# DavidSlayback/gym-po-taxi

Measured on AMD Instinct MI355X. Metric: env steps/sec (whole node), FourRooms 11x11 Hansen-4 at 1M envs, 1/2/4/8 GPUs, higher is better.
Workload: dtype int32; 1 GPU; configs[1]: FourRooms 11x11 (FR_MAP) Hansen-4 obs, 1048576 envs per GPU, MultistoryFourRoomsEnv(grid_z=1, obs_type='hansen'); envs_per_gpu=1048576, global_envs=1048576, rng_mode=numpy, parallelism=independent env shards x1, steps_per_launch_call=128, kernel_autotune=windowed

## Files before the change

### gym-po-taxi_amd/csrc/api.hip

```cpp
#include <stdarg.h>
#include <stdio.h>
#include <string.h>

#include <string>
#include <vector>

#include "gp_internal.h"

struct gp_env {
  int kind = 0;
  std::unique_ptr<EnvBackend> be;
};

static thread_local char g_err[1024] = "";

void gp_set_error(const char* fmt, ...) {
  va_list ap;
  va_start(ap, fmt);
  vsnprintf(g_err, sizeof(g_err), fmt, ap);
  va_end(ap);
}

const char* gp_derr_text(uint32_t flags) {
  static thread_local char buf[512];
// ... 184 lines not shown
  else if (!strcmp(key, "fault_block")) g_dbg.fault_block = (int)value;
  else if (!strcmp(key, "fused_tile")) g_dbg.fused_tile = (int)value;
  else if (!strcmp(key, "generic_kernels")) g_dbg.generic_kernels = value != 0;
  else if (!strcmp(key, "no_spw")) g_dbg.no_spw = value != 0;
  else if (!strcmp(key, "no_wgrid")) g_dbg.no_wgrid = value != 0;
  else if (!strcmp(key, "wg_halo")) g_dbg.wg_halo = (int)value;
  else if (!strcmp(key, "wg_bias")) g_dbg.wg_bias = (int)value;
  else if (!strcmp(key, "wg_tmode")) g_dbg.wg_tmode = (int)value;
  else if (!strcmp(key, "wg_kmax")) g_dbg.wg_kmax = (int)value;
  else if (!strcmp(key, "taxi_npg_min")) g_dbg.taxi_npg_min = (int)value;
  else if (!strcmp(key, "xg_min_envs")) g_dbg.xg_min_envs = (int)value;
  else if (!strcmp(key, "fused_step")) g_dbg.fused_step = value;
  else if (!strcmp(key, "wg_block_envs")) g_dbg.wg_block_envs = (int)value;
  else if (!strcmp(key, "wg_fill_simd")) g_dbg.wg_fill_simd = (int)value;
  else if (!strcmp(key, "wg_fill_wave")) g_dbg.wg_fill_wave = value;
  else if (!strcmp(key, "xg_ppt_min")) g_dbg.xg_ppt_min = (int)value;
  else if (!strcmp(key, "xg_spb_min")) g_dbg.xg_spb_min = (int)value;
  else if (!strcmp(key, "persist_bpc")) g_dbg.persist_bpc = (int)value;
  else if (!strcmp(key, "ctrl_lds_max")) g_dbg.ctrl_lds_max = (int)value;
  else if (!strcmp(key, "xg_graph")) gp_xg_graph_knob = (int)value;
  else {
    gp_set_error("gp_debug_set: unknown key '%s'", key);
    return GP_E_INVALID;
  }
  return GP_OK;
}
void gp_debug_reset(void) {
  g_dbg = GpDebugKnobs{};
  gp_xg_graph_knob = -1;
}
// ... 339 lines not shown
```

### gym-po-taxi_amd/csrc/gp_internal.h

```cpp
#pragma once
#include <cstring>
#include <memory>
#include <string>
#include <vector>

#include "../../include/gym_po_amd.h"
#include "gp_common.h"

struct RngHost {
  u128 state = 0, inc = 1;
  uint32_t has_u32 = 0, uinteger = 0;
};

std::vector<uint64_t> seed_sequence_u64(const std::vector<uint32_t>& entropy, const std::vector<uint32_t>& spawn_key,
                                        int n_words64);
RngHost pcg64_from_seed(const std::vector<uint32_t>& entropy, const std::vector<uint32_t>& spawn_key);
std::vector<double> argmax_multinomial_distribution(int m, int n);
std::vector<PcgJump> build_jump_tables(u128 inc);

struct GpDebugKnobs {
  int disable_fused = 0, no_staging = 0, xmode = 1, fault_block = -1;
  int fused_tile = 0;
  uint32_t spin_limit = 0;
  int generic_kernels = 0;
  int no_spw = 0;
  int no_wgrid = 0;
  int wg_halo = 0;
  int wg_bias = 0;
  int wg_tmode = 0;
  int wg_kmax = -1;
  int xg_min_envs = -1;
  int xg_ppt_min = -1;
  int xg_spb_min = -1;
  int taxi_npg_min = -1;
  int64_t fused_step = -1;
  int wg_block_envs = 0;
  int wg_fill_simd = 0;
  int64_t wg_fill_wave = 0;
  int ctrl_lds_max = -1;
  int persist_bpc = 0;
};
const GpDebugKnobs& gp_debug_knobs();

inline int persistent_grid(int ntiles, int cus, int occ) {
  const int forced = gp_debug_knobs().persist_bpc;
  const int bpc = forced > 0 ? forced : (occ < 1 ? 1 : (occ > 8 ? 8 : occ));
  const int g = cus * bpc;
  return ntiles < g ? (ntiles > 0 ? ntiles : 1) : g;
}

struct KernelTimer {
  bool on = false;
  std::vector<std::pair<hipEvent_t, hipEvent_t>> ev;
// ... 130 lines not shown
```

### gym-po-taxi_amd/csrc/grid.hip

```cpp
#include <stdarg.h>
#include <stdio.h>
#include <stdlib.h>
#include <string.h>

#include <algorithm>
#include <cmath>

#include "gp_ctrl.h"
#include "gp_internal.h"
#include "grid_shared.h"

namespace {

constexpr int TPB = 256;
constexpr int EPT = 4;
constexpr int EPB = TPB * EPT;
constexpr uint32_t SPIN_LIMIT = 1u << 24;
constexpr int MAX_TPB2 = 1024;
#ifndef WG_KMAX
#define WG_KMAX 24
#endif
#ifndef WG_FILL_WAVE
#define WG_FILL_WAVE 0xFFFF1111u
#endif
// ... 2513 lines not shown
  uint64_t philox_step = 0;
  std::vector<int32_t> cells;
  std::vector<uint16_t> goal_valid_h, agent_valid_h;
  DevBuf b_move, b_thr, b_gv, b_av, b_hbase, b_doff, b_hvec, b_t1, b_t2, b_coords, b_window, b_jt, b_lt4, b_lt2,
      b_tja, b_tjw, b_ae, b_goal, b_ctl, b_tcount, b_tlist, b_rflag, b_mslot, b_ftj, b_flt4, b_fjB, b_fslot, b_dbg, b_self, b_jt8,
      b_limg, b_ofix, b_avo;
  int fused_G = 0, fused_qpt = 0;
  int wg_G = 0, wg_E = 0, wg_NS = 0, wg_H = 0;
  int wg_kmax = WG_KMAX;
  int wg_kmax_default = WG_KMAX;
  size_t wg_lds = 0;
  int at_launches = 0, at_steps = 0;
  float at_ms[2] = {0.f, 0.f};
  WgParams wg{};
  std::vector<char> wg_img;
  DevBuf b_wgp, b_wlimg, b_wjlane, b_wjrej, b_wjblk, b_wslots, b_wjfirst;
  bool fused_stg = false;
  const uint64_t* rp_u = nullptr;
  const int32_t* rp_goal = nullptr;
  const int32_t* rp_agent = nullptr;

  int build(const gp_grid_config* cfg);
  int upload_rng();
  int refresh_lds_image();
  int seed(const RngHost& r, const uint32_t key[2]) override {
    rng = r;
    philox_key[0] = key[0];
    philox_key[1] = key[1];
    d.key0 = key[0];
    d.key1 = key[1];
    philox_step = 0;
// ... 6 lines not shown
  int get_rng_state(RngHost* r) override;
  int check() override;
  int device_error(uint32_t flags);
  int query(const char* key, int64_t* v) const override {
    if (!strcmp(key, "fused_blocks")) *v = fused_G;
    else if (!strcmp(key, "fused_tiles_per_block")) *v = fused_qpt;
    else if (!strcmp(key, "fused_staged")) *v = fused_stg ? 1 : 0;
    else if (!strcmp(key, "fused_spw")) *v = d.spw_on;
    else if (!strcmp(key, "fused_tile_envs")) *v = d.ftile;
    else if (!strcmp(key, "wgrid")) *v = wg_G > 0 ? 1 : 0;
    else if (!strcmp(key, "wgrid_blocks")) *v = wg_G;
    else if (!strcmp(key, "wgrid_block_envs")) *v = wg_E;
    else if (!strcmp(key, "wgrid_halo")) *v = wg_H;
    else if (!strcmp(key, "wgrid_kmax")) *v = wg_kmax;
    else if (!strcmp(key, "wgrid_lds")) *v = (int64_t)wg_lds;
    else if (!strcmp(key, "autotune_launches")) *v = at_launches;
    else if (!strcmp(key, "autotune_steps")) *v = at_steps;
    else if (!strcmp(key, "autotune_wgrid_ns")) *v = (int64_t)(at_ms[0] * 1e6f);
    else if (!strcmp(key, "autotune_fused_ns")) *v = (int64_t)(at_ms[1] * 1e6f);
    else if (!strcmp(key, "philox_step")) *v = (int64_t)philox_step;
    else if (!strcmp(key, "controller_nodes")) *v = ctrl.M;
    else if (!strcmp(key, "controller_lds")) *v = ctrl.M && ctrl.lds_off >= 0;
    else return EnvBackend::query(key, v);
    return GP_OK;
  }
  int reset(void* obs, hipStream_t s) override;
  int step(const void* act, void* obs, float* rew, uint8_t* term, uint8_t* trunc, hipStream_t s) override;
  int rollout(int K, const void* act, void* obs, float* rew, uint8_t* term, uint8_t* trunc, hipStream_t s) override;
  int get_state(void* a, void* b, void* c, void* dd, hipStream_t s) override {
    hipLaunchKernelGGL(grid_get_state, dim3((unsigned)((B + TPB - 1) / TPB)), dim3(TPB), 0, s, d, (int32_t*)a,
// ... 203 lines not shown
      E = e;
      break;
    }
  if (!E) return GP_OK;
  for (int c : ocell)
    if (c < INT32_MIN / 2 || c > INT32_MAX / 2) return GP_OK;
  const int H = dbg.wg_halo == 512 ? 512 : 256;
  const int nc = d.ncells, na = d.nact;
  WgLds L{};
  int off = 0;
  auto put = [&](int32_t& o, size_t bytes) {
    o = off;
    off += (int)((bytes + 15) / 16 * 16);
  };
  put(L.j32, sizeof(PcgJump) * 32);
  put(L.jt8, sizeof(PcgJump) * 512);
  put(L.move, (size_t)nc * na * 2);
  put(L.thr, (size_t)na * na * 8);
  put(L.ocell, (size_t)nc * 4);
  put(L.avalid, agent_valid_h.size() * 2);
  L.total = off;
  const size_t lds = (size_t)wg_dyn_bytes(L.total, E, H);
  if (!wgrid_fits(E / 512, na, lds)) return GP_OK;
  wg_img.assign((size_t)L.total, 0);
  memcpy(wg_img.data() + L.move, move.data(), move.size() * 2);
  std::vector<uint64_t> th(thr.size());
  for (size_t i = 0; i < thr.size(); ++i) th[i] = thr_on_u64(thr[i]);
  memcpy(wg_img.data() + L.thr, th.data(), th.size() * 8);
  memcpy(wg_img.data() + L.ocell, ocell.data(), ocell.size() * 4);
  memcpy(wg_img.data() + L.avalid, agent_valid_h.data(), agent_valid_h.size() * 2);
  wg_G = (int)(B / E);
  wg_E = E;
  wg_NS = E / 512;
  wg_H = H;
  wg_lds = lds;
  WgParams& w = wg;
  w.B = (int32_t)B;
// ... 32 lines not shown
      dv[v] = n >= 8 ? n - 16 : n;
      vsum += dv[v];
      vok = vok && base + dl[v & 3] + dv[v] >= 1;
    }
    if (vsum != 0 || !vok)
      for (int v = 0; v < 8; ++v) dv[v] = 0;
    int r = 0;
    for (int v = 0; v < 8; ++v) {
      w.fill_row0[v] = r;
      w.fill_rows[v] = base + dl[v & 3] + dv[v];
      r += w.fill_rows[v];
    }
  }
  w.wg_bias = dbg.wg_bias;
  w.tmode = dbg.wg_tmode;
  w.lds = L;
  int e;
  if ((e = b_wgp.alloc(sizeof(WgParams))) || (e = b_wlimg.alloc((size_t)L.total)) ||
      (e = b_wjlane.alloc(sizeof(PcgJump) * 1024)) || (e = b_wjrej.alloc(sizeof(PcgJump) * 64 * (size_t)wg_G)) ||
      (e = b_wjblk.alloc(sizeof(PcgJump) * 2 * (size_t)wg_G)) || (e = b_wslots.alloc(sizeof(uint64_t) * 4 * (size_t)wg_G)) ||
      (e = b_wjfirst.alloc(sizeof(PcgJump) * 1024)))
    return e;
  w.jfirst = b_wjfirst.as<PcgJump>();
  w.limg = b_wlimg.as<char>();
  w.jlane = b_wjlane.as<PcgJump>();
  w.jrej = b_wjrej.as<PcgJump>();
  w.jblk = b_wjblk.as<PcgJump>();
  w.slots = b_wslots.as<uint64_t>();
  return GP_OK;
}

int GridBackend::upload_wgrid() {
  const u128 inc = rng.inc;
  WgParams& w = wg;
  auto compose = [](const PcgJump& j2, const PcgJump& j1) {
    const u128 a = mk128(j2.a_hi, j2.a_lo) * mk128(j1.a_hi, j1.a_lo);
    const u128 c = mk128(j2.a_hi, j2.a_lo) * mk128(j1.c_hi, j1.c_lo) + mk128(j2.c_hi, j2.c_lo);
    return PcgJump{hi64(a), lo64(a), hi64(c), lo64(c)};
  };
  PcgJump* j32 = reinterpret_cast<PcgJump*>(wg_img.data() + w.lds.j32);
  PcgJump* jt8 = reinterpret_cast<PcgJump*>(wg_img.data() + w.lds.jt8);
  for (int i = 0; i < 32; ++i) j32[i] = pcg_jump_params((u128)i, inc);
  for (int i = 0; i < 256; ++i) {
    jt8[i] = pcg_jump_params((u128)i, inc);
    jt8[256 + i] = pcg_jump_params((u128)(256 * i), inc);
  }
  std::vector<PcgJump> jl(1024), jr((size_t)64 * wg_G), jb(2 * (size_t)wg_G);
  const PcgJump one = pcg_jump_params((u128)1, inc), j32s = pcg_jump_params((u128)32, inc);
  const PcgJump jBp1 = pcg_jump_params((u128)B + 1, inc);
  jl[1] = jBp1;
  for (int l = 1; l < 512; ++l) jl[2 * l + 1] = compose(j32s, jl[2 * (l - 1) + 1]);
  for (int v = 0; v < 8; ++v) {
    PcgJump x = pcg_jump_params((u128)(64 * w.fill_row0[v]), inc);
    for (int l = 0; l < 64; ++l) {
      jl[2 * (64 * v + l)] = x;
      x = compose(one, x);
    }
  }
  const PcgJump j62 = pcg_jump_params((u128)62, inc);
  PcgJump row = jBp1;
  for (int b = 0; b < wg_G; ++b) {
    PcgJump x = row;
    for (int l = 0; l < 64; ++l) {
      jr[(size_t)b * 64 + l] = x;
      x = compose(one, x);
    }
    row = compose(j62, row);
    jb[2 * b] = pcg_jump_params((u128)B + (u128)(b ? wg_E * b - wg_H : 0), inc);
    jb[2 * b + 1] = b ? pcg_jump_params((u128)(wg_E * b - wg_H + 1), inc) : PcgJump{0, 1, 0, 0};
  }
  w.jB = pcg_jump_params((u128)B, inc);
  w.jrow = pcg_jump_params((u128)64, inc);
  w.j512 = pcg_jump_params((u128)512, inc);
  std::vector<PcgJump> jf(1024);
  jf[0] = one;
  jf[512] = pcg_jump_params((u128)wg_H, inc);
  for (int l = 1; l < 512; ++l) {
    jf[l] = compose(one, jf[l - 1]);
    jf[512 + l] = compose(one, jf[512 + l - 1]);
  }
  w.jt64 = d.jt;
  w.dbg = d.dbg;
  w.ctl = d.ctl;
  w.mslot = d.mslot;
  w.ae = d.ae;
  GP_HIP_CHECK(hipMemcpy(b_wlimg.p, wg_img.data(), wg_img.size(), hipMemcpyHostToDevice));
  GP_HIP_CHECK(hipMemcpy(b_wjlane.p, jl.data(), jl.size() * sizeof(PcgJump), hipMemcpyHostToDevice));
  GP_HIP_CHECK(hipMemcpy(b_wjrej.p, jr.data(), jr.size() * sizeof(PcgJump), hipMemcpyHostToDevice));
  GP_HIP_CHECK(hipMemcpy(b_wjblk.p, jb.data(), jb.size() * sizeof(PcgJump), hipMemcpyHostToDevice));
  GP_HIP_CHECK(hipMemcpy(b_wjfirst.p, jf.data(), jf.size() * sizeof(PcgJump), hipMemcpyHostToDevice));
  GP_HIP_CHECK(hipMemcpy(b_wgp.p, &w, sizeof(WgParams), hipMemcpyHostToDevice));
  return GP_OK;
}

int GridBackend::get_rng_state(RngHost* r) {
  GP_HIP_CHECK(hipDeviceSynchronize());
  GridCtl c;
  GP_HIP_CHECK(hipMemcpy(&c, d.ctl, sizeof(c), hipMemcpyDeviceToHost));
  r->state = mk128(c.s_hi, c.s_lo);
  r->inc = mk128(c.inc_hi, c.inc_lo);
  r->has_u32 = c.has_u32;
  r->uinteger = c.uinteger;
  if (c.err) return device_error(c.err);
  return GP_OK;
// ... 737 lines not shown
```

### gym-po-taxi_amd/csrc/grid_shared.h

```cpp
#pragma once
#include "gp_common.h"

struct alignas(64) GridCtl {
  uint64_t s_hi, s_lo, inc_hi, inc_lo;
  uint32_t has_u32, uinteger;
  uint32_t epoch;
  uint32_t err;
  uint32_t b_total;
  uint32_t step;
  uint32_t fb_last;
  uint32_t wstep;
};

struct alignas(32) MetricSlot {
  double return_sum;
  unsigned long long episodes, length_sum, env_steps;
};

constexpr int WG_HMAX = 512;

struct WgLds {
  int32_t j32, jt8, move, thr, ocell, avalid, total;
};

struct WgParams {
  int32_t B, G, E, NS;
  int32_t nact, ncells, n_agent, goal;
  uint32_t thr_agent;
  int32_t time_limit, halo;
  float r_step, r_wall, r_goal;
  uint32_t spin_limit;
  int32_t fault_block;
  int32_t rw_words;
  int32_t fill_row0[8], fill_rows[8];
  int32_t wg_bias;
  int32_t tmode;
  WgLds lds;
  const char* limg;
  const PcgJump* jlane;
  const PcgJump* jrej;
  const PcgJump* jblk;
  const PcgJump* jfirst;
  const PcgJump* jt64;
  PcgJump jB, jrow, j512;
  GridCtl* ctl;
  MetricSlot* mslot;
  uint32_t* ae;
  uint64_t* slots;
  unsigned long long* dbg;
};

struct WgArgs {
  const WgParams* P;
  int32_t K;
  const int32_t* act;
  int32_t* obs;
  float* rew;
  uint8_t* term;
  uint8_t* trunc;
};

__host__ __device__ constexpr int wg_dyn_bytes(int tables, int E, int H) {
#ifndef WG_NSTG
#define WG_NSTG 3
#endif
  return tables + (E + 2 * H) * 8 + 2 * 512 * 16 + WG_NSTG * E * 4;
}
int wgrid_launch(const WgArgs& a, int NS, int NA, int G, size_t dyn_lds, hipStream_t s);
int wgrid_fits(int NS, int NA, size_t dyn_lds);
```

### gym-po-taxi_amd/csrc/wgrid.hip

```cpp
#include <stdint.h>

#include "gp_internal.h"
#include "grid_shared.h"

namespace {

#ifdef GP_STAMPS
constexpr int ST_STEPS = 24, ST_SLOTS = 42;
__shared__ unsigned long long g_stamp[32 * 32 + 8];
#define WSTAMP(P, k, i)                                                                                  \
  do {                                                                                                   \
    if ((threadIdx.x & 63) == 0 && (k) < ST_STEPS) {                                                     \
      unsigned long long t_;                                                                             \
      asm volatile("s_memrealtime %0\n\ts_waitcnt lgkmcnt(0)" : "=s"(t_)::"memory");                     \
      g_stamp[(k) * ST_SLOTS + (i)] = t_;                                                                \
    }                                                                                                    \
  } while (0)
#define LSTAMP(P, i)                                                                                     \
  do {                                                                                                   \
    if ((threadIdx.x & 63) == 0) {                                                                       \
      unsigned long long t_;                                                                             \
      asm volatile("s_memrealtime %0\n\ts_waitcnt lgkmcnt(0)" : "=s"(t_)::"memory");                     \
      g_stamp[32 * 32 + (i)] = t_;                                                                       \
    }                                                                                                    \
// ... 37 lines not shown
constexpr int NCAND = 512;
constexpr uint32_t CAND_W = 192;

struct WgShared {
  uint64_t mask[8][EW];
  uint32_t trans_done;
  uint32_t cs_done;
  uint32_t r2s_done;
  uint32_t fill_done;
  uint32_t res_done;
  uint32_t st_done;
  uint32_t sx_ready;
  uint32_t sy_ready;
  uint32_t cells_done;
  uint32_t pro;
  uint64_t sx[2][2];
  uint64_t sy[2][2];
  uint64_t rw[2][2];
  int32_t rw_off[2];
  uint32_t fix[2];
  uint32_t R, h, u, nrp;
  uint32_t cbase;
  uint32_t rp[MAXRP];
  uint16_t r2s[4096];
  uint16_t cand[NCAND];
};

__device__ __forceinline__ void lds_barrier() {
  __builtin_amdgcn_fence(__ATOMIC_RELEASE, "workgroup", "local");
  __builtin_amdgcn_s_barrier();
// ... 47 lines not shown
}

__host__ __device__ __forceinline__ uint64_t thr_on_u64(uint64_t t) {
  return t >= (1ull << 53) ? ~0ull : ((t << 11) | 0x7FFull);
}

template <int NA>
__device__ __forceinline__ int32_t action_row(int32_t a, uint32_t* derr) {
  if (action_out_of_range(a, NA)) flag_bad_action(derr);
  if (a < 0) a += NA;
  return min(max(a, 0), NA - 1) * NA * 8;
}

struct Tabs {
  const PcgJump* j32p;
  const PcgJump* jt8p;
  const int32_t* ocp;
  const uint16_t* avp;
  const PcgJump* jt64;
  int32_t halo;
  __device__ __forceinline__ Tabs(const char* d, const WgParams& P)
      : j32p(reinterpret_cast<const PcgJump*>(d + P.lds.j32)), jt8p(reinterpret_cast<const PcgJump*>(d + P.lds.jt8)),
        ocp(reinterpret_cast<const int32_t*>(d + P.lds.ocell)), avp(reinterpret_cast<const uint16_t*>(d + P.lds.avalid)),
        jt64(P.jt64), halo(P.halo) {}
  __device__ __forceinline__ const PcgJump& j32(uint32_t i) const { return j32p[i]; }
  __device__ __forceinline__ const PcgJump& jt8(uint32_t i) const { return jt8p[i]; }
  __device__ __forceinline__ int32_t ocell(uint32_t c) const { return ocp[c]; }
  __device__ __forceinline__ uint32_t avalid(uint32_t v) const { return avp[v]; }
};

__device__ __forceinline__ u128 load_cs(const uint64_t* CS, uint32_t j) {
  const ulonglong2 v = reinterpret_cast<const ulonglong2*>(CS)[j];
  return mk128(v.y, v.x);
}
__device__ __forceinline__ u128 draw_state(const Tabs& tb, const uint64_t* CS, uint32_t d) {
  return apply_jump(tb.j32(d & 31u), load_cs(CS, d >> 5));
}

__device__ __forceinline__ u128 jump_any(const Tabs& tb, u128 s, uint32_t n) {
  if (n < 65536u) {
    if (n & 255u) s = apply_jump(tb.jt8(n & 255u), s);
    if (n >> 8) s = apply_jump(tb.jt8(256u + (n >> 8)), s);
    return s;
  }
  return pcg_jump(tb.jt64, s, n);
}

__device__ __forceinline__ u128 rw_base(const Tabs& tb, const PcgJump& jb, u128 Sx, uint32_t used, int beta,
                                        int32_t& heff) {
  const int32_t H = tb.halo;
  if (beta == 0) {
    heff = min(H, (int32_t)used + 1);
    return apply_jump(jb, jump_any(tb, Sx, used + 1u - (uint32_t)heff));
  }
  heff = H;
  return apply_jump(jb, jump_any(tb, Sx, used + 1u));
}
// ... 57 lines not shown
#define WG_NSTG 3
#endif
#ifndef WG_EAGER_TAIL
#define WG_EAGER_TAIL 4
#endif
#ifndef WG_SUNROLL
#define WG_SUNROLL 2
#endif
constexpr int NSTG = WG_NSTG;
struct Lds {
  uint64_t* RW;
  uint64_t* CS0;
  char* stg0;
  __device__ __forceinline__ Lds(char* dyn, const WgParams& P, int E)
      : RW(reinterpret_cast<uint64_t*>(dyn + P.lds.total)),
        CS0(reinterpret_cast<uint64_t*>(dyn + P.lds.total + (size_t)(E + 2 * P.halo) * 8)),
        stg0(dyn + P.lds.total + (size_t)(E + 2 * P.halo) * 8 + 2 * 512 * 16) {}
  __device__ __forceinline__ char* stg(int k, int E) const { return stg0 + (size_t)(k % NSTG) * E * 4; }
  __device__ __forceinline__ uint64_t* CS(int k) const { return CS0 + (size_t)(k & 1) * 1024; }
};

__device__ __forceinline__ void list_slice(const WgParams& P, WgShared& sh, const Tabs& tb, const uint64_t* CS,
                                           uint32_t sigma, u128 Sy, uint32_t h, uint32_t u) {
  const int lane = threadIdx.x & 63;
  bool rlo = false, rhi = false;
  if (lane < SLICE) {
    const uint32_t d = 62u * sigma + (uint32_t)lane;
    const u128 s = d < 16384u ? draw_state(tb, CS, d) : pcg_jump(tb.jt64, Sy, d + 1u);
    const uint64_t x = pcg_output(s);
    rlo = lemire_rejected((uint32_t)x, (uint32_t)P.n_agent, P.thr_agent);
    rhi = lemire_rejected((uint32_t)(x >> 32), (uint32_t)P.n_agent, P.thr_agent);
  }
// ... 57 lines not shown
    uint64_t g[4];
    exchange(P, slots + (size_t)(r & 1u) * G, (ts << 6) | r, cnt, 0u, g);
    rtot += list_flagged(P, sh, tb, CS, g, r, Sy, h, u);
    covered += 124u * (uint32_t)G;
  }
  uint32_t wtot = 0;
  if (b) {
    uint32_t p = b - 1u;
    const uint32_t n = sh.nrp;
    for (uint32_t q = 0; q < n; ++q) p += sh.rp[q] <= p ? 1u : 0u;
    wtot = p + 1u;
  }
  return wtot;
}

template <int NS, int NA>
__device__ __forceinline__ void wg_ctrl(const WgParams& P, WgShared& sh, const Tabs& tb, const Lds& L, int K) {
  const int lane = threadIdx.x & 63, beta = (int)blockIdx.x, G = (int)gridDim.x;
  constexpr int E = NS * 512;
  GridCtl* C = P.ctl;
  u128 Sx = mk128(C->s_hi, C->s_lo);
  uint32_t h = C->has_u32, u = C->uinteger;
  uint32_t bprev = C->fb_last;
  uint32_t Rprev = (uint32_t)(((uint64_t)bprev * (uint64_t)blockIdx.x) / (uint64_t)gridDim.x);
  const uint32_t ts0 = C->wstep + 1u;
  const PcgJump jr = P.jrej[(size_t)beta * 64 + lane];
  const PcgJump jb = P.jblk[2 * beta], jpro = P.jblk[2 * beta + 1];
  const PcgJump jB = P.jB;
  const uint32_t nag = (uint32_t)P.n_agent, thra = P.thr_agent;
  const int32_t H = P.halo;
  const uint32_t bias = (uint32_t)P.wg_bias;
  const bool envcells = NS <= 2 && !(P.tmode & TM_CELLSWAP);
  uint32_t* derr = &C->err;
  lds_barrier();
  if (lane == 0 && (P.tmode & TM_OLDPRO)) {
    const u128 s = apply_jump(jpro, Sx);
    sh.rw[0][0] = hi64(s);
    sh.rw[0][1] = lo64(s);
    sh.rw_off[0] = beta == 0 ? 1 : H;
    lds_release();
    __hip_atomic_store(&sh.pro, 1u, __ATOMIC_RELAXED, __HIP_MEMORY_SCOPE_WORKGROUP);
  }
  LSTAMP(P, 1);
  for (int k = 0; k < K; ++k) {
    const uint32_t ts = ts0 + (uint32_t)k;
    if (lane == 0) {
      sh.sx[k & 1][0] = hi64(Sx);
      sh.sx[k & 1][1] = lo64(Sx);
      lds_release();
      __hip_atomic_store(&sh.sx_ready, (uint32_t)k + 1u, __ATOMIC_RELAXED, __HIP_MEMORY_SCOPE_WORKGROUP);
    }
    uint32_t rj = 0;
    if (lane < SLICE) {
      const uint64_t x = pcg_output(apply_jump(jr, Sx));
      rj = (lemire_rejected((uint32_t)x, nag, thra) ? 1u : 0u) + (lemire_rejected((uint32_t)(x >> 32), nag, thra) ? 1u : 0u);
    } else if (lane == SLICE && beta == 0 && h) {
      rj = lemire_rejected(u, nag, thra) ? 1u : 0u;
    }
    const uint32_t rejc = wave_sum(rj);
    WSTAMP(P, k, 6);
    lds_wait(&sh.trans_done, (uint32_t)EW * (uint32_t)(k + 1), derr);
    WSTAMP(P, k, 7);
    const uint32_t cb = wave_sum(lane < NS * EW ? (uint32_t)__builtin_popcountll(sh.mask[lane >> 3][lane & 7]) : 0u);
    uint64_t* slots = P.slots + (size_t)(ts & 1u) * 2 * G;
    publish(P, slots, ts << 6, rejc, cb);
    WSTAMP(P, k, 8);
    const u128 Sy = apply_jump(jB, Sx);
    uint32_t used_p, hp;
    words_to_draws(bprev + bias, h, used_p, hp);
    int32_t heff_p;
    const u128 Srw = rw_base(tb, jb, Sx, used_p, beta, heff_p);
    if (lane == 0) {
      sh.sy[k & 1][0] = hi64(Sy);
      sh.sy[k & 1][1] = lo64(Sy);
      sh.rw[(k + 1) & 1][0] = hi64(Srw);
      sh.rw[(k + 1) & 1][1] = lo64(Srw);
      lds_release();
      __hip_atomic_store(&sh.sy_ready, (uint32_t)k + 1u, __ATOMIC_RELAXED, __HIP_MEMORY_SCOPE_WORKGROUP);
    }
    const uint64_t* CS = L.CS(k);
    lds_wait(&sh.cs_done, (uint32_t)EW * (uint32_t)(k + 1), derr);
    const uint32_t d0 = min(Rprev > CAND_W + h ? (Rprev - CAND_W - h) >> 1 : 0u, 16384u - NCAND / 2);
    const uint32_t cbase = 2u * d0 + h;
    if (!(P.tmode & TM_NOCAND)) {
#pragma unroll
      for (int m = 0; m < NCAND / 128; ++m) {
        const uint32_t j = (uint32_t)(lane + 64 * m);
        const uint64_t x = pcg_output(draw_state(tb, CS, d0 + j));
        sh.cand[2 * j] = (uint16_t)tb.avalid(lemire_value((uint32_t)x, nag));
        sh.cand[2 * j + 1] = (uint16_t)tb.avalid(lemire_value((uint32_t)(x >> 32), nag));
      }
// ... 47 lines not shown
            cell = tb.avalid(lemire_value(word, nag));
          }
          st[2 * slot] = (uint16_t)cell;
        }
      }
    } else {
      const uint32_t wtot = ctrl_slow(P, sh, tb, CS, Sy, h, u, b, ts, g);
      words_to_draws(wtot, h, used, h2);
      if (lane == 0) {
        sh.R = R;
        sh.h = h;
        sh.u = u;
      }
    }
    int32_t off = heff_p + (int32_t)used - (int32_t)used_p;
    uint32_t fix = slow ? 1u : 0u;
    if (k + 1 < K && (off < 0 || off > 2 * H)) {
      int32_t heff;
      const u128 s = rw_base(tb, jb, Sx, used, beta, heff);
      off = heff;
      fix |= 2u;
      if (lane == 0) {
        sh.rw[(k + 1) & 1][0] = hi64(s);
        sh.rw[(k + 1) & 1][1] = lo64(s);
      }
    }
    if (lane == 0) {
      sh.rw_off[(k + 1) & 1] = off;
      sh.fix[k & 1] = fix;
      lds_release();
      __hip_atomic_store(&sh.cells_done, (uint32_t)k + 1u, __ATOMIC_RELAXED, __HIP_MEMORY_SCOPE_WORKGROUP);
    }
    WSTAMP(P, k, 10);
    Sx = jump_any(tb, Sy, used);
    if (used) u = (uint32_t)(pcg_output(Sx) >> 32);
    h = h2;
    bprev = b;
    Rprev = R;
    WSTAMP(P, k, 12);
  }
  LSTAMP(P, 3);
  if (beta == 0 && lane == 0) {
    C->s_hi = hi64(Sx);
    C->s_lo = lo64(Sx);
    C->has_u32 = h;
    C->uinteger = u;
    C->fb_last = bprev;
    C->wstep = ts0 + (uint32_t)K - 1u;
  }
}

struct Acc {
  uint32_t eps = 0, ngoal = 0, nwall = 0, lens = 0;
};

template <int NS>
__device__ __forceinline__ void wg_env_slow(const WgParams& P, WgShared& sh, const Tabs& tb, const uint64_t* CS,
                                            int k, char* stg, uint32_t dn, const uint32_t (&pre)[NS],
                                            const uint64_t (&bm)[NS], uint32_t (&ae)[NS]) {
  const int lg = threadIdx.x;
  const u128 Sy = mk128(sh.sy[k & 1][0], sh.sy[k & 1][1]);
  const uint32_t R = sh.R, h = sh.h, u = sh.u, n = sh.nrp;
#pragma unroll
// ... 45 lines not shown
    reinterpret_cast<uint16_t*>(stg)[2 * (s * 512 + lg)] = (uint16_t)cell;
    ae[s] = cell;
  }
}

__device__ __forceinline__ void fill_window(uint64_t* RW, const PcgJump& jl, const PcgJump& jrow, int fr0, int nrow,
                                            u128 base, int lane) {
  u128 s = apply_jump(jl, base);
  uint64_t* d = RW + fr0 * 64 + lane;
  for (int m = 0; m < nrow; ++m) {
    d[m * 64] = pcg_output(s);
    s = apply_jump(jrow, s);
  }
}

template <int NS, int NA>
__device__ __forceinline__ void wg_env(const WgParams& P, WgShared& sh, const Tabs& tb, const Lds& L, const char* dyn,
                                       const int32_t* __restrict__ act, int K, Acc& acc, int32_t* __restrict__ obs,
                                       float* __restrict__ rew, uint8_t* __restrict__ term,
                                       uint8_t* __restrict__ trunc) {
  const int lg = threadIdx.x, lane = lg & 63, w = lg >> 6;
  const int beta = (int)blockIdx.x, G = (int)gridDim.x;
  constexpr int E = NS * 512;
  const size_t B = (size_t)E * (size_t)G;
  const size_t e0 = (size_t)beta * E;
  const char* thr = dyn + P.lds.thr;
  const char* mv = dyn + P.lds.move;
  const uint32_t goal = (uint32_t)P.goal, tlim = (uint32_t)P.time_limit;
  uint32_t* derr = &P.ctl->err;
  uint32_t* aeg = P.ae;
  const bool envcells = NS <= 2 && !(P.tmode & TM_CELLSWAP);
// ... 27 lines not shown
    }
  }
  if (w == 0) LSTAMP(P, 2);
  lds_barrier();
#pragma unroll
  for (int k = 0; k < NS; ++k) {
    arow[k] = action_row<NA>(anext[k], derr);
    acc.lens += ae[k] >> 16;
  }
  if (oldpro) {
    lds_wait(&sh.pro, 1u, derr);
    if (lane == 0) lds_add(&sh.fill_done, 1u);
  }
  if (w == 0) LSTAMP(P, 7);
  uint32_t fill_target = EW;
  uint64_t bm[NS];
  uint32_t pre[NS];
  for (int k = 0; k < K; ++k) {
    char* stg = L.stg(k, E);
    if (w == 0) WSTAMP(P, k, 41);
    if (k + 1 < K && !(tmode & (TM_LATEACT | TM_ACTSTART))) {
#pragma unroll
      for (int s = 0; s < NS; ++s) anext[s] = act[(size_t)(k + 1) * B + e0 + (size_t)s * 512 + lg];
    }
    if (w == 0) WSTAMP(P, k, 40);
    lds_wait(&sh.fill_done, fill_target, derr);
    if (k >= NSTG) lds_wait(&sh.st_done, (uint32_t)SW * (uint32_t)(k - NSTG + 1), derr);
    if (!(tmode & TM_NOPRIO)) __builtin_amdgcn_s_setprio(2);
    if (w == 0) WSTAMP(P, k, 0);
    WSTAMP(P, k, 32 + w);
    if (k + 1 < K && (tmode & TM_ACTSTART)) {
#pragma unroll
      for (int s = 0; s < NS; ++s) anext[s] = act[(size_t)(k + 1) * B + e0 + (size_t)s * 512 + lg];
    }
    const int32_t off = sh.rw_off[k & 1];
    uint32_t dn = 0;
    uint32_t mvo[NS];
#pragma unroll
    for (int s = 0; s < NS; ++s) {
      const uint64_t x = L.RW[s * 512 + lg + off];
      const char* t = thr + arow[s];
      uint32_t eb = 0;
#pragma unroll
      for (int j = 0; j + 1 < NA; j += 2) {
        const ulonglong2 tt = *reinterpret_cast<const ulonglong2*>(t + 8 * j);
        eb = x > tt.x ? (uint32_t)(2 * (j + 1)) : eb;
        if (j + 2 < NA) eb = x > tt.y ? (uint32_t)(2 * (j + 2)) : eb;
      }
      mvo[s] = (ae[s] & 0xFFFFu) * (2 * NA) + eb;
    }
    uint32_t mm[NS];
#pragma unroll
    for (int s = 0; s < NS; ++s) mm[s] = *reinterpret_cast<const uint16_t*>(mv + mvo[s]);
    uint32_t sv[NS];
#pragma unroll
// ... 35 lines not shown
    if (lane == 0) lds_add(&sh.cs_done, 1u);
    if (w == 0) WSTAMP(P, k, 3);
    lds_wait(&sh.trans_done, (uint32_t)EW * (uint32_t)(k + 1), derr);
    {
      const uint32_t c = lane < NS * EW ? (uint32_t)__builtin_popcountll(sh.mask[lane >> 3][lane & 7]) : 0u;
      const uint32_t ex = wave_incl_scan(c) - c;
#pragma unroll
      for (int s = 0; s < NS; ++s) {
        pre[s] = (uint32_t)__builtin_amdgcn_readlane((int)ex, s * EW + w);
        if ((dn >> s) & 1u) sh.r2s[pre[s] + mbcnt(bm[s])] = (uint16_t)(s * 512 + lg);
      }
    }
    lds_release();
    if (lane == 0) lds_add(&sh.r2s_done, 1u);
    if (w == 0) WSTAMP(P, k, 4);
    if (k + 1 < K) {
      lds_wait(&sh.sy_ready, (uint32_t)k + 1u, derr);
      const u128 Srw = mk128(sh.rw[(k + 1) & 1][0], sh.rw[(k + 1) & 1][1]);
      if (!(tmode & TM_NOFILL)) fill_window(L.RW, jrw, jrow, fr0, nrow, Srw, lane);
      lds_release();
      if (lane == 0) lds_add(&sh.fill_done, 1u);
      fill_target += EW;
#pragma unroll
      for (int s = 0; s < NS; ++s) arow[s] = action_row<NA>(anext[s], derr);
    }
    if (w == 0) WSTAMP(P, k, 5);
    if (w == EW - 1) WSTAMP(P, k, 15);
    WSTAMP(P, k, 24 + w);
    lds_wait(&sh.cells_done, (uint32_t)k + 1u, derr);
    if (w == 0) WSTAMP(P, k, 11);
    const uint32_t fix = sh.fix[k & 1];
// ... 10 lines not shown
    if (lane == 0) lds_add(&sh.res_done, 1u);
    if (k == K - 1 && !(tmode & TM_NOSTORE)) {
      const uint32_t* st = reinterpret_cast<const uint32_t*>(stg);
      const size_t base = (size_t)k * B + e0 + (size_t)lg;
#pragma unroll
      for (int s = 0; s < NS; ++s) {
        const uint32_t v = st[s * 512 + lg];
        const size_t e = base + (size_t)s * 512;
        obs[e] = tb.ocell(v & 0xFFFFu);
        rew[e] = (v & 0x10000u) ? P.r_goal : ((v & 0x40000u) ? P.r_wall : P.r_step);
        term[e] = (uint8_t)((v >> 16) & 1u);
        trunc[e] = (uint8_t)((v >> 17) & 1u);
      }
    }
    if ((fix & 2u) && k + 1 < K) {
      fill_window(L.RW, jrw, jrow, fr0, nrow, mk128(sh.rw[(k + 1) & 1][0], sh.rw[(k + 1) & 1][1]), lane);
      lds_release();
      if (lane == 0) lds_add(&sh.fill_done, 1u);
      fill_target += EW;
    }
  }
#pragma unroll
  for (int k = 0; k < NS; ++k) {
    aeg[e0 + (size_t)k * 512 + lg] = ae[k];
    acc.lens -= ae[k] >> 16;
  }
}

typedef uint32_t u32x4 __attribute__((ext_vector_type(4)));
__device__ __forceinline__ void nt_store(void* p, u32x4 v) { __builtin_nontemporal_store(v, reinterpret_cast<u32x4*>(p)); }

template <int NS>
__device__ __forceinline__ void wg_store(const WgParams& P, WgShared& sh, const Tabs& tb, const Lds& L, int K,
                                         int32_t* __restrict__ obs, float* __restrict__ rew, uint8_t* __restrict__ term,
// ... 70 lines not shown
      v0 = s[i0];
      if (a1) v1 = s[i0 + CT];
      if (a2) v2 = s[i0 + 2 * CT];
      if (a3) v3 = s[i0 + 3 * CT];
      d[i0] = v0;
      if (a1) d[i0 + CT] = v1;
      if (a2) d[i0 + 2 * CT] = v2;
      if (a3) d[i0 + 3 * CT] = v3;
    }
    if (wid == EW) LSTAMP(P, 5);
    if (wid == EW + 1) LSTAMP(P, 6);
  }
  if (tid == EW * 64) {
    sh.trans_done = sh.cs_done = sh.r2s_done = sh.fill_done = sh.res_done = sh.st_done = 0;
    sh.sx_ready = sh.sy_ready = sh.cells_done = sh.pro = 0;
    if (!(P.tmode & TM_OLDPRO)) sh.fill_done = EW;
    sh.fix[0] = sh.fix[1] = 0;
  }
  const Tabs tb(dyn, P);
  const Lds L(dyn, P, E);
  Acc acc;
  if (wid == CWAVE) {
    __builtin_amdgcn_s_setprio(3);
    wg_ctrl<NS, NA>(P, sh, tb, L, K);
  } else if (wid > CWAVE) {
    if (P.tmode & TM_STORELOW) __builtin_amdgcn_s_setprio(0);
    else __builtin_amdgcn_s_setprio(1);
    wg_store<NS>(P, sh, tb, L, K, obs, rew, term, trunc);
  } else {
    wg_env<NS, NA>(P, sh, tb, L, dyn, act, K, acc, obs, rew, term, trunc);
  }
  float rsum = 0.f;
  uint32_t nst = 0;
  if (wid < EW) {
    const uint32_t steps = (uint32_t)(NS * K);
    acc.lens += steps;
    nst = steps;
    rsum = (float)acc.ngoal * P.r_goal + (float)acc.nwall * P.r_wall + (float)(steps - acc.ngoal - acc.nwall) * P.r_step;
  }
#pragma unroll
  for (int d = 32; d >= 1; d >>= 1) {
    rsum += __shfl_xor(rsum, d, 64);
    acc.eps += __shfl_xor(acc.eps, d, 64);
    acc.lens += __shfl_xor(acc.lens, d, 64);
    nst += __shfl_xor(nst, d, 64);
// ... 80 lines not shown
```

Baseline: 192.8 billion env-steps/s.

## Add opt-in two-step-ahead random window prefill with double-buffered LDS windows

Adds an optional mode where env waves prefill the random-word window for step k+2 while step k runs. It uses two LDS windows, a planner wave, and a regeneration path for when the window prediction misses. This aims to hide window-fill latency behind the step computation, at the cost of extra LDS and more synchronisation. The default path also shrinks the PCG jump table from two 8-bit levels to three 6-bit levels. That saves LDS but can add a third jump application per lookup.

```diff
diff --git a/gym-po-taxi_amd/csrc/api.hip b/gym-po-taxi_amd/csrc/api.hip
--- a/gym-po-taxi_amd/csrc/api.hip
+++ b/gym-po-taxi_amd/csrc/api.hip
@@ -222,6 +222,7 @@
   else if (!strcmp(key, "wg_block_envs")) g_dbg.wg_block_envs = (int)value;
   else if (!strcmp(key, "wg_fill_simd")) g_dbg.wg_fill_simd = (int)value;
   else if (!strcmp(key, "wg_fill_wave")) g_dbg.wg_fill_wave = value;
+  else if (!strcmp(key, "wg_ahead")) g_dbg.wg_ahead = (int)value;
   else if (!strcmp(key, "xg_ppt_min")) g_dbg.xg_ppt_min = (int)value;
   else if (!strcmp(key, "xg_spb_min")) g_dbg.xg_spb_min = (int)value;
   else if (!strcmp(key, "persist_bpc")) g_dbg.persist_bpc = (int)value;
diff --git a/gym-po-taxi_amd/csrc/gp_internal.h b/gym-po-taxi_amd/csrc/gp_internal.h
--- a/gym-po-taxi_amd/csrc/gp_internal.h
+++ b/gym-po-taxi_amd/csrc/gp_internal.h
@@ -37,6 +37,7 @@
   int wg_block_envs = 0;
   int wg_fill_simd = 0;
   int64_t wg_fill_wave = 0;
+  int wg_ahead = 0;
   int ctrl_lds_max = -1;
   int persist_bpc = 0;
 };
diff --git a/gym-po-taxi_amd/csrc/grid.hip b/gym-po-taxi_amd/csrc/grid.hip
--- a/gym-po-taxi_amd/csrc/grid.hip
+++ b/gym-po-taxi_amd/csrc/grid.hip
@@ -2551,7 +2551,7 @@
   float at_ms[2] = {0.f, 0.f};
   WgParams wg{};
   std::vector<char> wg_img;
-  DevBuf b_wgp, b_wlimg, b_wjlane, b_wjrej, b_wjblk, b_wslots, b_wjfirst;
+  DevBuf b_wgp, b_wlimg, b_wjlane, b_wjrej, b_wjblk, b_wjblk2, b_wslots, b_wjfirst;
   bool fused_stg = false;
   const uint64_t* rp_u = nullptr;
   const int32_t* rp_goal = nullptr;
@@ -2588,6 +2588,13 @@
     else if (!strcmp(key, "wgrid_halo")) *v = wg_H;
     else if (!strcmp(key, "wgrid_kmax")) *v = wg_kmax;
     else if (!strcmp(key, "wgrid_lds")) *v = (int64_t)wg_lds;
+    else if (!strcmp(key, "wgrid_ahead")) *v = wg_G ? wg.ahead : 0;
+    else if (!strcmp(key, "wgrid_regen")) {
+      GridCtl c;
+      GP_HIP_CHECK(hipDeviceSynchronize());
+      GP_HIP_CHECK(hipMemcpy(&c, d.ctl, sizeof(GridCtl), hipMemcpyDeviceToHost));
+      *v = c.wregen;
+    }
     else if (!strcmp(key, "autotune_launches")) *v = at_launches;
     else if (!strcmp(key, "autotune_steps")) *v = at_steps;
     else if (!strcmp(key, "autotune_wgrid_ns")) *v = (int64_t)(at_ms[0] * 1e6f);
@@ -2821,13 +2828,18 @@
     off += (int)((bytes + 15) / 16 * 16);
   };
   put(L.j32, sizeof(PcgJump) * 32);
-  put(L.jt8, sizeof(PcgJump) * 512);
+  put(L.jt, sizeof(PcgJump) * 144);
   put(L.move, (size_t)nc * na * 2);
   put(L.thr, (size_t)na * na * 8);
   put(L.ocell, (size_t)nc * 4);
   put(L.avalid, agent_valid_h.size() * 2);
   L.total = off;
-  const size_t lds = (size_t)wg_dyn_bytes(L.total, E, H);
+  int ahead = dbg.wg_ahead == 2 ? 2 : 1;
+  size_t lds = (size_t)wg_dyn_bytes(L.total, E, H, ahead);
+  if (ahead == 2 && !wgrid_fits(E / 512, na, lds)) {
+    ahead = 1;
+    lds = (size_t)wg_dyn_bytes(L.total, E, H, 1);
+  }
   if (!wgrid_fits(E / 512, na, lds)) return GP_OK;
   wg_img.assign((size_t)L.total, 0);
   memcpy(wg_img.data() + L.move, move.data(), move.size() * 2);
@@ -2890,13 +2902,15 @@
   }
   w.wg_bias = dbg.wg_bias;
   w.tmode = dbg.wg_tmode;
+  w.ahead = ahead;
   w.lds = L;
   int e;
   if ((e = b_wgp.alloc(sizeof(WgParams))) || (e = b_wlimg.alloc((size_t)L.total)) ||
       (e = b_wjlane.alloc(sizeof(PcgJump) * 1024)) || (e = b_wjrej.alloc(sizeof(PcgJump) * 64 * (size_t)wg_G)) ||
       (e = b_wjblk.alloc(sizeof(PcgJump) * 2 * (size_t)wg_G)) || (e = b_wslots.alloc(sizeof(uint64_t) * 4 * (size_t)wg_G)) ||
-      (e = b_wjfirst.alloc(sizeof(PcgJump) * 1024)))
+      (e = b_wjfirst.alloc(sizeof(PcgJump) * 1024)) || (e = b_wjblk2.alloc(sizeof(PcgJump) * (size_t)wg_G)))
     return e;
+  w.jblk2 = b_wjblk2.as<PcgJump>();
   w.jfirst = b_wjfirst.as<PcgJump>();
   w.limg = b_wlimg.as<char>();
   w.jlane = b_wjlane.as<PcgJump>();
@@ -2915,13 +2929,14 @@
     return PcgJump{hi64(a), lo64(a), hi64(c), lo64(c)};
   };
   PcgJump* j32 = reinterpret_cast<PcgJump*>(wg_img.data() + w.lds.j32);
-  PcgJump* jt8 = reinterpret_cast<PcgJump*>(wg_img.data() + w.lds.jt8);
+  PcgJump* jt = reinterpret_cast<PcgJump*>(wg_img.data() + w.lds.jt);
   for (int i = 0; i < 32; ++i) j32[i] = pcg_jump_params((u128)i, inc);
-  for (int i = 0; i < 256; ++i) {
-    jt8[i] = pcg_jump_params((u128)i, inc);
-    jt8[256 + i] = pcg_jump_params((u128)(256 * i), inc);
-  }
-  std::vector<PcgJump> jl(1024), jr((size_t)64 * wg_G), jb(2 * (size_t)wg_G);
+  for (int i = 0; i < 64; ++i) {
+    jt[i] = pcg_jump_params((u128)i, inc);
+    jt[64 + i] = pcg_jump_params((u128)(64 * i), inc);
+    if (i < 16) jt[128 + i] = pcg_jump_params((u128)(4096 * i), inc);
+  }
+  std::vector<PcgJump> jl(1024), jr((size_t)64 * wg_G), jb(2 * (size_t)wg_G), jb2((size_t)wg_G);
   const PcgJump one = pcg_jump_params((u128)1, inc), j32s = pcg_jump_params((u128)32, inc);
   const PcgJump jBp1 = pcg_jump_params((u128)B + 1, inc);
   jl[1] = jBp1;
@@ -2944,6 +2959,7 @@
     row = compose(j62, row);
     jb[2 * b] = pcg_jump_params((u128)B + (u128)(b ? wg_E * b - wg_H : 0), inc);
     jb[2 * b + 1] = b ? pcg_jump_params((u128)(wg_E * b - wg_H + 1), inc) : PcgJump{0, 1, 0, 0};
+    jb2[b] = pcg_jump_params((u128)(2 * B + (int64_t)wg_E * b - wg_H), inc);
   }
   w.jB = pcg_jump_params((u128)B, inc);
   w.jrow = pcg_jump_params((u128)64, inc);
@@ -2964,6 +2980,7 @@
   GP_HIP_CHECK(hipMemcpy(b_wjlane.p, jl.data(), jl.size() * sizeof(PcgJump), hipMemcpyHostToDevice));
   GP_HIP_CHECK(hipMemcpy(b_wjrej.p, jr.data(), jr.size() * sizeof(PcgJump), hipMemcpyHostToDevice));
   GP_HIP_CHECK(hipMemcpy(b_wjblk.p, jb.data(), jb.size() * sizeof(PcgJump), hipMemcpyHostToDevice));
+  GP_HIP_CHECK(hipMemcpy(b_wjblk2.p, jb2.data(), jb2.size() * sizeof(PcgJump), hipMemcpyHostToDevice));
   GP_HIP_CHECK(hipMemcpy(b_wjfirst.p, jf.data(), jf.size() * sizeof(PcgJump), hipMemcpyHostToDevice));
   GP_HIP_CHECK(hipMemcpy(b_wgp.p, &w, sizeof(WgParams), hipMemcpyHostToDevice));
   return GP_OK;
diff --git a/gym-po-taxi_amd/csrc/grid_shared.h b/gym-po-taxi_amd/csrc/grid_shared.h
--- a/gym-po-taxi_amd/csrc/grid_shared.h
+++ b/gym-po-taxi_amd/csrc/grid_shared.h
@@ -10,6 +10,7 @@
   uint32_t step;
   uint32_t fb_last;
   uint32_t wstep;
+  uint32_t wregen;
 };
 
 struct alignas(32) MetricSlot {
@@ -20,7 +21,7 @@
 constexpr int WG_HMAX = 512;
 
 struct WgLds {
-  int32_t j32, jt8, move, thr, ocell, avalid, total;
+  int32_t j32, jt, move, thr, ocell, avalid, total;
 };
 
 struct WgParams {
@@ -35,11 +36,13 @@
   int32_t fill_row0[8], fill_rows[8];
   int32_t wg_bias;
   int32_t tmode;
+  int32_t ahead;
   WgLds lds;
   const char* limg;
   const PcgJump* jlane;
   const PcgJump* jrej;
   const PcgJump* jblk;
+  const PcgJump* jblk2;
   const PcgJump* jfirst;
   const PcgJump* jt64;
   PcgJump jB, jrow, j512;
@@ -60,11 +63,11 @@
   uint8_t* trunc;
 };
 
-__host__ __device__ constexpr int wg_dyn_bytes(int tables, int E, int H) {
+__host__ __device__ constexpr int wg_dyn_bytes(int tables, int E, int H, int nwin) {
 #ifndef WG_NSTG
 #define WG_NSTG 3
 #endif
-  return tables + (E + 2 * H) * 8 + 2 * 512 * 16 + WG_NSTG * E * 4;
+  return tables + nwin * (E + 2 * H) * 8 + 2 * 512 * 16 + WG_NSTG * E * 4;
 }
 int wgrid_launch(const WgArgs& a, int NS, int NA, int G, size_t dyn_lds, hipStream_t s);
 int wgrid_fits(int NS, int NA, size_t dyn_lds);
diff --git a/gym-po-taxi_amd/csrc/wgrid.hip b/gym-po-taxi_amd/csrc/wgrid.hip
--- a/gym-po-taxi_amd/csrc/wgrid.hip
+++ b/gym-po-taxi_amd/csrc/wgrid.hip
@@ -75,6 +75,11 @@
   uint32_t sy_ready;
   uint32_t cells_done;
   uint32_t pro;
+  uint32_t wfill[2];
+  uint32_t regen_done;
+  uint32_t rwb_ready;
+  uint64_t rwb[4][2];
+  uint32_t ph[2], pb[2];
   uint64_t sx[2][2];
   uint64_t sy[2][2];
   uint64_t rw[2][2];
@@ -152,17 +157,17 @@
 
 struct Tabs {
   const PcgJump* j32p;
-  const PcgJump* jt8p;
+  const PcgJump* jtp;
   const int32_t* ocp;
   const uint16_t* avp;
   const PcgJump* jt64;
   int32_t halo;
   __device__ __forceinline__ Tabs(const char* d, const WgParams& P)
-      : j32p(reinterpret_cast<const PcgJump*>(d + P.lds.j32)), jt8p(reinterpret_cast<const PcgJump*>(d + P.lds.jt8)),
+      : j32p(reinterpret_cast<const PcgJump*>(d + P.lds.j32)), jtp(reinterpret_cast<const PcgJump*>(d + P.lds.jt)),
         ocp(reinterpret_cast<const int32_t*>(d + P.lds.ocell)), avp(reinterpret_cast<const uint16_t*>(d + P.lds.avalid)),
         jt64(P.jt64), halo(P.halo) {}
   __device__ __forceinline__ const PcgJump& j32(uint32_t i) const { return j32p[i]; }
-  __device__ __forceinline__ const PcgJump& jt8(uint32_t i) const { return jt8p[i]; }
+  __device__ __forceinline__ const PcgJump& jt(uint32_t i) const { return jtp[i]; }
   __device__ __forceinline__ int32_t ocell(uint32_t c) const { return ocp[c]; }
   __device__ __forceinline__ uint32_t avalid(uint32_t v) const { return avp[v]; }
 };
@@ -177,8 +182,9 @@
 
 __device__ __forceinline__ u128 jump_any(const Tabs& tb, u128 s, uint32_t n) {
   if (n < 65536u) {
-    if (n & 255u) s = apply_jump(tb.jt8(n & 255u), s);
-    if (n >> 8) s = apply_jump(tb.jt8(256u + (n >> 8)), s);
+    if (n & 63u) s = apply_jump(tb.jt(n & 63u), s);
+    if ((n >> 6) & 63u) s = apply_jump(tb.jt(64u + ((n >> 6) & 63u)), s);
+    if (n >> 12) s = apply_jump(tb.jt(128u + (n >> 12)), s);
     return s;
   }
   return pcg_jump(tb.jt64, s, n);
@@ -266,8 +272,9 @@
   char* stg0;
   __device__ __forceinline__ Lds(char* dyn, const WgParams& P, int E)
       : RW(reinterpret_cast<uint64_t*>(dyn + P.lds.total)),
-        CS0(reinterpret_cast<uint64_t*>(dyn + P.lds.total + (size_t)(E + 2 * P.halo) * 8)),
-        stg0(dyn + P.lds.total + (size_t)(E + 2 * P.halo) * 8 + 2 * 512 * 16) {}
+        CS0(reinterpret_cast<uint64_t*>(dyn + P.lds.total + (size_t)P.ahead * (E + 2 * P.halo) * 8)),
+        stg0(dyn + P.lds.total + (size_t)P.ahead * (E + 2 * P.halo) * 8 + 2 * 512 * 16) {}
+  __device__ __forceinline__ uint64_t* win(int j, int E, int H) const { return RW + (size_t)(j & 1) * (E + 2 * H); }
   __device__ __forceinline__ char* stg(int k, int E) const { return stg0 + (size_t)(k % NSTG) * E * 4; }
   __device__ __forceinline__ uint64_t* CS(int k) const { return CS0 + (size_t)(k & 1) * 1024; }
 };
@@ -355,7 +362,7 @@
   return wtot;
 }
 
-template <int NS, int NA>
+template <int NS, int NA, bool A2>
 __device__ __forceinline__ void wg_ctrl(const WgParams& P, WgShared& sh, const Tabs& tb, const Lds& L, int K) {
   const int lane = threadIdx.x & 63, beta = (int)blockIdx.x, G = (int)gridDim.x;
   constexpr int E = NS * 512;
@@ -368,6 +375,8 @@
   const PcgJump jr = P.jrej[(size_t)beta * 64 + lane];
   const PcgJump jb = P.jblk[2 * beta], jpro = P.jblk[2 * beta + 1];
   const PcgJump jB = P.jB;
+  uint32_t n1 = 0, n2 = 0, usedprev = 0, nregen = 0;
+  int32_t heff1 = P.halo;
   const uint32_t nag = (uint32_t)P.n_agent, thra = P.thr_agent;
   const int32_t H = P.halo;
   const uint32_t bias = (uint32_t)P.wg_bias;
@@ -388,6 +397,8 @@
     if (lane == 0) {
       sh.sx[k & 1][0] = hi64(Sx);
       sh.sx[k & 1][1] = lo64(Sx);
+      sh.ph[k & 1] = h;
+      sh.pb[k & 1] = bprev;
       lds_release();
       __hip_atomic_store(&sh.sx_ready, (uint32_t)k + 1u, __ATOMIC_RELAXED, __HIP_MEMORY_SCOPE_WORKGROUP);
     }
@@ -407,15 +418,30 @@
     publish(P, slots, ts << 6, rejc, cb);
     WSTAMP(P, k, 8);
     const u128 Sy = apply_jump(jB, Sx);
-    uint32_t used_p, hp;
-    words_to_draws(bprev + bias, h, used_p, hp);
-    int32_t heff_p;
-    const u128 Srw = rw_base(tb, jb, Sx, used_p, beta, heff_p);
+    uint32_t used_p = 0, hp;
+    int32_t heff_p = 0;
+    u128 Srw = Sy;
+    if (!A2) {
+      words_to_draws(bprev + bias, h, used_p, hp);
+      Srw = rw_base(tb, jb, Sx, used_p, beta, heff_p);
+    }
+    if (A2) {
+      uint32_t upa, hpa, upb, hpb;
+      words_to_draws(bprev + bias, h, upa, hpa);
+      words_to_draws(bprev + bias, hpa, upb, hpb);
+      if (k == 0) {
+        n1 = upa + 1u;
+        heff1 = beta == 0 ? min(H, (int32_t)upa + 1) : H;
+      }
+      n2 = upa + upb + 1u;
+    }
     if (lane == 0) {
       sh.sy[k & 1][0] = hi64(Sy);
       sh.sy[k & 1][1] = lo64(Sy);
-      sh.rw[(k + 1) & 1][0] = hi64(Srw);
-      sh.rw[(k + 1) & 1][1] = lo64(Srw);
+      if (!A2) {
+        sh.rw[(k + 1) & 1][0] = hi64(Srw);
+        sh.rw[(k + 1) & 1][1] = lo64(Srw);
+      }
       lds_release();
       __hip_atomic_store(&sh.sy_ready, (uint32_t)k + 1u, __ATOMIC_RELAXED, __HIP_MEMORY_SCOPE_WORKGROUP);
     }
@@ -493,12 +519,19 @@
       }
     }
     int32_t off = heff_p + (int32_t)used - (int32_t)used_p;
+    bool miss = off < 0 || off > 2 * H;
+    if (A2) {
+      const int64_t o = (int64_t)heff1 + (int64_t)usedprev + (int64_t)used + 1 - (int64_t)n1;
+      miss = o < 0 || o > 2 * H;
+      off = miss ? 0 : (int32_t)o;
+    }
     uint32_t fix = slow ? 1u : 0u;
-    if (k + 1 < K && (off < 0 || off > 2 * H)) {
+    if (k + 1 < K && miss) {
       int32_t heff;
       const u128 s = rw_base(tb, jb, Sx, used, beta, heff);
       off = heff;
       fix |= 2u;
+      ++nregen;
       if (lane == 0) {
         sh.rw[(k + 1) & 1][0] = hi64(s);
         sh.rw[(k + 1) & 1][1] = lo64(s);
@@ -516,6 +549,9 @@
     h = h2;
     bprev = b;
     Rprev = R;
+    usedprev = used;
+    n1 = n2;
+    heff1 = H;
     WSTAMP(P, k, 12);
   }
   LSTAMP(P, 3);
@@ -526,6 +562,7 @@
     C->uinteger = u;
     C->fb_last = bprev;
     C->wstep = ts0 + (uint32_t)K - 1u;
+    C->wregen = nregen;
   }
 }
 
@@ -601,7 +638,77 @@
   }
 }
 
-template <int NS, int NA>
+constexpr int PLANW = 3;
+__device__ __forceinline__ void wg_plan(const WgParams& P, WgShared& sh, const Tabs& tb, int k, int K) {
+  const int lane = threadIdx.x & 63, beta = (int)blockIdx.x;
+  const u128 Sx = mk128(sh.sx[k & 1][0], sh.sx[k & 1][1]);
+  const uint32_t h = sh.ph[k & 1], bp = sh.pb[k & 1] + (uint32_t)P.wg_bias;
+  uint32_t upa, hpa, upb, hpb;
+  words_to_draws(bp, h, upa, hpa);
+  words_to_draws(bp, hpa, upb, hpb);
+  if (k == 0 && K > 1) {
+    int32_t heff;
+    const u128 s1 = rw_base(tb, P.jblk[2 * beta], Sx, upa, beta, heff);
+    if (lane == 0) {
+      sh.rwb[1][0] = hi64(s1);
+      sh.rwb[1][1] = lo64(s1);
+    }
+  }
+  if (k + 2 < K) {
+    const u128 s2 = apply_jump(P.jblk2[beta], jump_any(tb, Sx, upa + upb + 1u));
+    if (lane == 0) {
+      sh.rwb[(k + 2) & 3][0] = hi64(s2);
+      sh.rwb[(k + 2) & 3][1] = lo64(s2);
+    }
+  }
+  if (lane == 0) {
+    lds_release();
+    __hip_atomic_store(&sh.rwb_ready, (uint32_t)min(k + 2, K - 1), __ATOMIC_RELAXED, __HIP_MEMORY_SCOPE_WORKGROUP);
+  }
+}
+
+struct FillTask {
+  int fw = 1, fr = 0;
+  u128 s = 0;
+};
+__device__ __forceinline__ void fill_task(WgShared& sh, const Lds& L, FillTask& f, const PcgJump& jl, const PcgJump& jrow,
+                                          int fr0, int nrow, int lane, int E, int H, int upto, uint32_t stop, int due,
+                                          bool nofill, bool prio, uint32_t* derr) {
+  uint32_t cd = stop ? lds_load(&sh.cells_done) : 0u;
+  while (f.fw <= upto) {
+    if (prio) {
+      if (f.fw <= due) __builtin_amdgcn_s_setprio(2);
+      else __builtin_amdgcn_s_setprio(0);
+    }
+    if (f.fr == 0) {
+      if (stop) {
+        while (lds_load(&sh.rwb_ready) < (uint32_t)f.fw) {
+          if (lds_load(&sh.cells_done) >= stop) return;
+          __builtin_amdgcn_s_sleep(1);
+        }
+      }
+      lds_wait(&sh.rwb_ready, (uint32_t)f.fw, derr);
+      f.s = apply_jump(jl, mk128(sh.rwb[f.fw & 3][0], sh.rwb[f.fw & 3][1]));
+      if (nofill) f.fr = nrow;
+    }
+    uint64_t* d = L.win(f.fw, E, H) + fr0 * 64 + lane;
+    while (f.fr < nrow) {
+      if (stop) {
+        if (cd >= stop) return;
+        cd = lds_load(&sh.cells_done);
+      }
+      d[f.fr * 64] = pcg_output(f.s);
+      f.s = apply_jump(jrow, f.s);
+      ++f.fr;
+    }
+    lds_release();
+    if (lane == 0) lds_add(&sh.wfill[f.fw & 1], 1u);
+    ++f.fw;
+    f.fr = 0;
+  }
+}
+
+template <int NS, int NA, bool A2>
 __device__ __forceinline__ void wg_env(const WgParams& P, WgShared& sh, const Tabs& tb, const Lds& L, const char* dyn,
                                        const int32_t* __restrict__ act, int K, Acc& acc, int32_t* __restrict__ obs,
                                        float* __restrict__ rew, uint8_t* __restrict__ term,
@@ -659,6 +766,11 @@
   }
   if (w == 0) LSTAMP(P, 7);
   uint32_t fill_target = EW;
+  FillTask ft;
+  uint32_t regen_target = 0;
+  const int32_t H = P.halo;
+  const bool nofill = (tmode & TM_NOFILL) != 0;
+  const bool fprio = !(tmode & (TM_NOPRIO | TM_ENVHIGH));
   uint64_t bm[NS];
   uint32_t pre[NS];
   for (int k = 0; k < K; ++k) {
@@ -670,6 +782,12 @@
     }
     if (w == 0) WSTAMP(P, k, 40);
     lds_wait(&sh.fill_done, fill_target, derr);
+    if (A2) {
+      fill_task(sh, L, ft, jrw, jrow, fr0, nrow, lane, E, H, k, 0u, k, nofill, fprio, derr);
+      lds_wait(&sh.wfill[k & 1], (uint32_t)EW * (uint32_t)((k + 1) >> 1), derr);
+      lds_wait(&sh.regen_done, regen_target, derr);
+    }
+    const uint64_t* RWk = A2 ? L.win(k, E, H) : L.RW;
     if (k >= NSTG) lds_wait(&sh.st_done, (uint32_t)SW * (uint32_t)(k - NSTG + 1), derr);
     if (!(tmode & TM_NOPRIO)) __builtin_amdgcn_s_setprio(2);
     if (w == 0) WSTAMP(P, k, 0);
@@ -683,7 +801,7 @@
     uint32_t mvo[NS];
 #pragma unroll
     for (int s = 0; s < NS; ++s) {
-      const uint64_t x = L.RW[s * 512 + lg + off];
+      const uint64_t x = RWk[s * 512 + lg + off];
       const char* t = thr + arow[s];
       uint32_t eb = 0;
 #pragma unroll
@@ -749,7 +867,15 @@
     lds_release();
     if (lane == 0) lds_add(&sh.r2s_done, 1u);
     if (w == 0) WSTAMP(P, k, 4);
-    if (k + 1 < K) {
+    if (A2) {
+      if (w == PLANW) wg_plan(P, sh, tb, k, K);
+      fill_task(sh, L, ft, jrw, jrow, fr0, nrow, lane, E, H, min(k + 2, K - 1), (uint32_t)k + 1u, k + 1, nofill, fprio, derr);
+      if (fprio) __builtin_amdgcn_s_setprio(0);
+      if (k + 1 < K) {
+#pragma unroll
+        for (int s = 0; s < NS; ++s) arow[s] = action_row<NA>(anext[s], derr);
+      }
+    } else if (k + 1 < K) {
       lds_wait(&sh.sy_ready, (uint32_t)k + 1u, derr);
       const u128 Srw = mk128(sh.rw[(k + 1) & 1][0], sh.rw[(k + 1) & 1][1]);
       if (!(tmode & TM_NOFILL)) fill_window(L.RW, jrw, jrow, fr0, nrow, Srw, lane);
@@ -790,10 +916,22 @@
       }
     }
     if ((fix & 2u) && k + 1 < K) {
-      fill_window(L.RW, jrw, jrow, fr0, nrow, mk128(sh.rw[(k + 1) & 1][0], sh.rw[(k + 1) & 1][1]), lane);
-      lds_release();
-      if (lane == 0) lds_add(&sh.fill_done, 1u);
-      fill_target += EW;
+      if (A2) {
+        if (ft.fw == k + 1) {
+          if (lane == 0) lds_add(&sh.wfill[(k + 1) & 1], 1u);
+          ft.fw = k + 2;
+          ft.fr = 0;
+        }
+        fill_window(L.win(k + 1, E, H), jrw, jrow, fr0, nrow, mk128(sh.rw[(k + 1) & 1][0], sh.rw[(k + 1) & 1][1]), lane);
+        lds_release();
+        if (lane == 0) lds_add(&sh.regen_done, 1u);
+        regen_target += EW;
+      } else {
+        fill_window(L.RW, jrw, jrow, fr0, nrow, mk128(sh.rw[(k + 1) & 1][0], sh.rw[(k + 1) & 1][1]), lane);
+        lds_release();
+        if (lane == 0) lds_add(&sh.fill_done, 1u);
+        fill_target += EW;
+      }
     }
   }
 #pragma unroll
@@ -894,6 +1032,7 @@
   if (tid == EW * 64) {
     sh.trans_done = sh.cs_done = sh.r2s_done = sh.fill_done = sh.res_done = sh.st_done = 0;
     sh.sx_ready = sh.sy_ready = sh.cells_done = sh.pro = 0;
+    sh.wfill[0] = sh.wfill[1] = sh.regen_done = sh.rwb_ready = 0;
     if (!(P.tmode & TM_OLDPRO)) sh.fill_done = EW;
     sh.fix[0] = sh.fix[1] = 0;
   }
@@ -902,13 +1041,15 @@
   Acc acc;
   if (wid == CWAVE) {
     __builtin_amdgcn_s_setprio(3);
-    wg_ctrl<NS, NA>(P, sh, tb, L, K);
+    if (P.ahead == 2) wg_ctrl<NS, NA, true>(P, sh, tb, L, K);
+    else wg_ctrl<NS, NA, false>(P, sh, tb, L, K);
   } else if (wid > CWAVE) {
     if (P.tmode & TM_STORELOW) __builtin_amdgcn_s_setprio(0);
     else __builtin_amdgcn_s_setprio(1);
     wg_store<NS>(P, sh, tb, L, K, obs, rew, term, trunc);
   } else {
-    wg_env<NS, NA>(P, sh, tb, L, dyn, act, K, acc, obs, rew, term, trunc);
+    if (P.ahead == 2) wg_env<NS, NA, true>(P, sh, tb, L, dyn, act, K, acc, obs, rew, term, trunc);
+    else wg_env<NS, NA, false>(P, sh, tb, L, dyn, act, K, acc, obs, rew, term, trunc);
   }
   float rsum = 0.f;
   uint32_t nst = 0;
```

New measurement: 192.0 billion env-steps/s. No clear change (-0.4%).
